# NeuralRevenant/RASSEngine

Hardware: AMD Instinct MI355X
Metric: queries/sec, exact cosine top-10 over N x 1024-d fp32 corpus in HBM (higher is better)
Workload: dtype f32; 1 GPU; 1000000 x 1024-d flat cosine top-10, 1 x MI355X, precomputed embeddings (BASELINE configs[1]); rows_per_gpu=1000000, rows_global=1000000, dim=1024, k=10, query_batch=32, corpus_dtype=f32, layout=tile16, mode=flat

## Files before the change

### include/rass_engine.h

```cpp
#ifndef RASS_ENGINE_H
#define RASS_ENGINE_H

#include <stddef.h>
#include <stdint.h>

#ifdef __cplusplus
extern "C" {
#endif

#define RASS_ABI_VERSION 1

typedef enum rass_status {
    RASS_OK = 0,
    RASS_ERR_INVALID = -1,
    RASS_ERR_HIP = -2,
    RASS_ERR_OOM = -3,
    RASS_ERR_NOT_FOUND = -4,
    RASS_ERR_UNSUPPORTED = -5,
    RASS_ERR_IO = -6
} rass_status;

typedef enum rass_dtype {
    RASS_F32 = 0,
    RASS_BF16 = 1,
// ... 304 lines not shown
                         const int64_t* d_row_ids, int64_t n, int dim, float* d_out,
                         int64_t out_stride, void* stream);
int rass_compact_plan(const int32_t* d_tags, int64_t n_rows, int64_t* d_new_row,
                      int64_t* d_src_row, int64_t* d_n_live, void* d_workspace,
                      size_t workspace_bytes, void* stream);
size_t rass_compact_plan_workspace_bytes(int64_t n_rows);
int rass_compact_rows_f32(const float* d_src, float* d_dst, int64_t row_stride,
                          const int64_t* d_src_row, int64_t n_dst, int64_t n_src_rows,
                          void* stream);

int rass_scan_topk_f32(const float* d_corpus, int64_t n_rows, int dim,
                       int64_t row_stride, const int32_t* d_row_tag,
                       const float* d_queries, int nq,
                       const int32_t* d_q_filter, int k, int64_t id_base,
                       float* d_out_scores, int64_t* d_out_ids,
                       void* d_workspace, size_t workspace_bytes,
                       void* stream);

int rass_topk_merge(const float* d_scores, const int64_t* d_ids, int n_lists,
                    int nq, int k, float* d_out_scores, int64_t* d_out_ids,
                    void* stream);

int rass_topk_merge_strided(const float* d_scores, const int64_t* d_ids,
                            int64_t score_list_stride, int64_t id_list_stride,
                            int n_lists, int nq, int k, float* d_out_scores,
                            int64_t* d_out_ids, void* stream);

int rass_topk_merge_strided_batch(const float* d_scores, const int64_t* d_ids,
                                  int64_t score_list_stride, int64_t id_list_stride,
                                  int n_lists, int nq_total, int group_size,
                                  int64_t score_group_stride, int64_t id_group_stride, int k,
                                  float* d_out_scores, int64_t* d_out_ids, void* stream);

int rass_peer_buffer_create(int device, size_t bytes, void** d_ptr, unsigned char* handle64);
int rass_peer_buffer_open(int device, const unsigned char* handle64, void** d_ptr);
int rass_peer_buffer_close(void* d_ptr, int opened_from_handle);
int rass_peer_post(const void* d_record, size_t bytes, void* d_remote_slot, void* d_remote_flag,
                   uint64_t seq, void* stream);
int rass_peer_wait(const void* d_flags, int n, int flag_stride_bytes, uint64_t seq, int* d_status,
                   int64_t max_spins, void* stream);

int rass_normalize_rows_f32(const float* d_in, int64_t in_stride, float* d_out,
                            int64_t out_stride, int64_t n, int dim,
                            void* stream);

typedef struct rass_ivf rass_ivf_t;

int rass_kmeans_assign(rass_index_t* idx, int64_t first_block, int64_t block_step,
                       int64_t n_blocks, const float* d_centroids_tile16, int nlist,
                       int32_t* d_assign, float* d_best);
int rass_kmeans_accumulate(rass_index_t* idx, int64_t first_block, int64_t block_step,
                           int64_t n_blocks, const int32_t* d_assign, float* d_sums,
                           float* d_counts, int nlist);

int rass_ivf_build(rass_index_t* src, const float* centroids, int nlist,
                   const int32_t* assign, rass_ivf_t** out);
int rass_ivf_build_ex(rass_index_t* src, const float* centroids, int nlist,
                      const int32_t* assign, rass_dtype slab_dtype, rass_ivf_t** out);
void rass_ivf_destroy(rass_ivf_t* ivf);
int rass_ivf_save(rass_ivf_t* ivf, const char* path);
int rass_ivf_load(rass_engine_t* eng, const char* path, rass_ivf_t** out);
int64_t rass_ivf_rows(const rass_ivf_t* ivf);
int rass_ivf_nlist(const rass_ivf_t* ivf);
int rass_ivf_dtype(const rass_ivf_t* ivf);
int rass_ivf_search(rass_ivf_t* ivf, const float* queries, int nq, int k,
                    int nprobe, const int32_t* q_filter, float* out_scores,
// ... 140 lines not shown
```

### rassengine_amd/_native.py

```python
from __future__ import annotations

import ctypes
import os
from typing import Optional

_HERE = os.path.dirname(os.path.abspath(__file__))
LIB_PATH = os.environ.get("RASS_HIP_LIB") or os.path.join(_HERE, "lib", "librass_hip.so")

RASS_OK = 0
RASS_MAX_K = 32
RASS_MAX_K_MULTIPASS = 4096
RASS_TAG_PATIENT_MASK = 0x00FFFFFF
RASS_TAG_DOCTYPE_SHIFT = 24
RASS_TAG_DOCTYPE_MASK = 0x7F000000
RASS_MAX_QBATCH = 32
RASS_MAX_DEVICE_BATCH = 4096
RASS_MAX_MMR_FETCH = 128
RASS_F32 = 0
RASS_BF16 = 1
RASS_QFILTER_NONE = -1
RASS_MAX_ATTRS = 8
RASS_ATTR_MISSING = -(1 << 31)
RASS_MAX_ATTR_CLAUSES = 64
RASS_ATTR_ALL, RASS_ATTR_ANY = 0, 1
# ... 170 lines not shown
                                                      ctypes.c_void_p, ctypes.c_void_p, ctypes.c_void_p]),
    "rass_index_step_floors_device": (ctypes.c_int, [ctypes.c_void_p, ctypes.c_void_p, ctypes.c_int, ctypes.c_int,
                                                     ctypes.c_void_p, ctypes.c_void_p]),
    "rass_index_save": (ctypes.c_int, [ctypes.c_void_p, ctypes.c_char_p]),
    "rass_index_load": (ctypes.c_int, [ctypes.c_void_p, ctypes.c_char_p, ctypes.c_char_p, c_void_pp]),
    "rass_index_fill_synthetic": (ctypes.c_int, [ctypes.c_void_p, ctypes.c_int64, ctypes.c_uint64,
                                                 ctypes.c_int64]),
    "rass_scan_workspace_bytes": (ctypes.c_size_t, [ctypes.c_int, ctypes.c_int]),
    "rass_scan_topk_f32": (ctypes.c_int, [ctypes.c_void_p, ctypes.c_int64, ctypes.c_int, ctypes.c_int64,
                                          ctypes.c_void_p, ctypes.c_void_p, ctypes.c_int, ctypes.c_void_p,
                                          ctypes.c_int, ctypes.c_int64, ctypes.c_void_p, ctypes.c_void_p,
                                          ctypes.c_void_p, ctypes.c_size_t, ctypes.c_void_p]),
    "rass_pack_rows_f32": (ctypes.c_int, [ctypes.c_void_p, ctypes.c_int64, ctypes.c_void_p, ctypes.c_int64,
                                          ctypes.c_int64, ctypes.c_int64, ctypes.c_int, ctypes.c_int,
                                          ctypes.c_void_p]),
    "rass_unpack_rows_f32": (ctypes.c_int, [ctypes.c_void_p, ctypes.c_int64, ctypes.c_int64, ctypes.c_int64,
                                            ctypes.c_int, ctypes.c_void_p, ctypes.c_int64, ctypes.c_void_p]),
    "rass_gather_rows_f32": (ctypes.c_int, [ctypes.c_void_p, ctypes.c_int64, ctypes.c_int64, ctypes.c_void_p, ctypes.c_int64,
                                            ctypes.c_int, ctypes.c_void_p, ctypes.c_int64, ctypes.c_void_p]),
    "rass_compact_plan": (ctypes.c_int, [ctypes.c_void_p, ctypes.c_int64, ctypes.c_void_p, ctypes.c_void_p, ctypes.c_void_p,
                                         ctypes.c_void_p, ctypes.c_size_t, ctypes.c_void_p]),
    "rass_compact_plan_workspace_bytes": (ctypes.c_size_t, [ctypes.c_int64]),
    "rass_compact_rows_f32": (ctypes.c_int, [ctypes.c_void_p, ctypes.c_void_p, ctypes.c_int64, ctypes.c_void_p, ctypes.c_int64,
                                             ctypes.c_int64, ctypes.c_void_p]),
    "rass_topk_merge": (ctypes.c_int, [ctypes.c_void_p, ctypes.c_void_p, ctypes.c_int, ctypes.c_int, ctypes.c_int,
                                       ctypes.c_void_p, ctypes.c_void_p, ctypes.c_void_p]),
    "rass_topk_merge_strided": (ctypes.c_int, [ctypes.c_void_p, ctypes.c_void_p, ctypes.c_int64, ctypes.c_int64,
                                               ctypes.c_int, ctypes.c_int, ctypes.c_int, ctypes.c_void_p,
                                               ctypes.c_void_p, ctypes.c_void_p]),
    "rass_topk_merge_strided_batch": (ctypes.c_int, [ctypes.c_void_p, ctypes.c_void_p, ctypes.c_int64, ctypes.c_int64,
                                                     ctypes.c_int, ctypes.c_int, ctypes.c_int, ctypes.c_int64,
                                                     ctypes.c_int64, ctypes.c_int, ctypes.c_void_p, ctypes.c_void_p,
                                                     ctypes.c_void_p]),
    "rass_normalize_rows_f32": (ctypes.c_int, [ctypes.c_void_p, ctypes.c_int64, ctypes.c_void_p, ctypes.c_int64,
                                               ctypes.c_int64, ctypes.c_int, ctypes.c_void_p]),
    "rass_peer_buffer_create": (ctypes.c_int, [ctypes.c_int, ctypes.c_size_t, c_void_pp, ctypes.c_char_p]),
    "rass_peer_buffer_open": (ctypes.c_int, [ctypes.c_int, ctypes.c_char_p, c_void_pp]),
    "rass_peer_buffer_close": (ctypes.c_int, [ctypes.c_void_p, ctypes.c_int]),
    "rass_peer_post": (ctypes.c_int, [ctypes.c_void_p, ctypes.c_size_t, ctypes.c_void_p, ctypes.c_void_p,
                                      ctypes.c_uint64, ctypes.c_void_p]),
    "rass_peer_wait": (ctypes.c_int, [ctypes.c_void_p, ctypes.c_int, ctypes.c_int, ctypes.c_uint64, ctypes.c_void_p,
                                      ctypes.c_int64, ctypes.c_void_p]),
    "rass_kmeans_assign": (ctypes.c_int, [ctypes.c_void_p, ctypes.c_int64, ctypes.c_int64, ctypes.c_int64,
                                          ctypes.c_void_p, ctypes.c_int, ctypes.c_void_p, ctypes.c_void_p]),
    "rass_kmeans_accumulate": (ctypes.c_int, [ctypes.c_void_p, ctypes.c_int64, ctypes.c_int64, ctypes.c_int64,
                                              ctypes.c_void_p, ctypes.c_void_p, ctypes.c_void_p, ctypes.c_int]),
    "rass_ivf_save": (ctypes.c_int, [ctypes.c_void_p, ctypes.c_char_p]),
    "rass_ivf_load": (ctypes.c_int, [ctypes.c_void_p, ctypes.c_char_p, c_void_pp]),
    "rass_ivf_build": (ctypes.c_int, [ctypes.c_void_p, ctypes.c_void_p, ctypes.c_int, ctypes.c_void_p, c_void_pp]),
    "rass_ivf_destroy": (None, [ctypes.c_void_p]),
    "rass_ivf_build_ex": (ctypes.c_int, [ctypes.c_void_p, ctypes.c_void_p, ctypes.c_int, ctypes.c_void_p, ctypes.c_int,
                                         c_void_pp]),
    "rass_ivf_dtype": (ctypes.c_int, [ctypes.c_void_p]),
    "rass_ivf_rows": (ctypes.c_int64, [ctypes.c_void_p]),
    "rass_ivf_nlist": (ctypes.c_int, [ctypes.c_void_p]),
    "rass_ivf_search": (ctypes.c_int, [ctypes.c_void_p, ctypes.c_void_p, ctypes.c_int, ctypes.c_int, ctypes.c_int,
                                       ctypes.c_void_p, ctypes.c_void_p, ctypes.c_void_p, c_i64_p]),
    "rass_ivf_search_device": (ctypes.c_int, [ctypes.c_void_p, ctypes.c_void_p, ctypes.c_int, ctypes.c_int,
                                              ctypes.c_int, ctypes.c_void_p, ctypes.c_void_p, ctypes.c_void_p]),
    "rass_ivf_search_device_batch": (ctypes.c_int, [ctypes.c_void_p, ctypes.c_void_p, ctypes.c_int, ctypes.c_int,
                                                    ctypes.c_int, ctypes.c_void_p, ctypes.c_void_p, ctypes.c_void_p,
                                                    ctypes.c_void_p]),
    "rass_ivf_build_prefix": (ctypes.c_int, [ctypes.c_void_p, ctypes.c_void_p, ctypes.c_int, ctypes.c_void_p, ctypes.c_int,
                                             ctypes.c_int64, c_void_pp]),
    "rass_ivf_covered_rows": (ctypes.c_int64, [ctypes.c_void_p]),
    "rass_ivf_delete": (ctypes.c_int, [ctypes.c_void_p, ctypes.c_int64]),
# ... 127 lines not shown
```

### rassengine_amd/csrc/api.hip

```cpp

#include "api_internal.h"

namespace rass {
namespace host {

thread_local std::string g_err;

int fail(int code, const std::string& msg) {
    g_err = msg;
    (void)hipGetLastError();
    return code;
}


int hip_fail(hipError_t e, const char* expr, const char* file, int line) {
    char b[512];
    snprintf(b, sizeof(b), "%s failed: %s (%s:%d)", expr, hipGetErrorString(e), file, line);
    return fail(e == hipErrorOutOfMemory ? RASS_ERR_OOM : RASS_ERR_HIP, b);
}

int check_nq(int nq) {
    return nq < 1 || nq > RASS_MAX_QBATCH ? fail(RASS_ERR_INVALID, "nq must be in [1, RASS_MAX_QBATCH]") : RASS_OK;
}
int check_k(int k) { return k < 1 || k > RASS_MAX_K ? fail(RASS_ERR_INVALID, "k must be in [1, RASS_MAX_K]") : RASS_OK; }
// ... 899 lines not shown
    if ((int64_t)n_lists * k > rass::kMergeMaxCandidates)
        return fail(RASS_ERR_UNSUPPORTED, "n_lists * k exceeds 8192 candidates");
    HIP_TRY(rass::launch_merge_topk(d_scores, d_ids, n_lists, nq, k, d_out_scores, d_out_ids,
                                    reinterpret_cast<hipStream_t>(stream), nullptr, score_list_stride,
                                    id_list_stride));
    return RASS_OK;
}

int rass_topk_merge_strided_batch(const float* d_scores, const int64_t* d_ids, int64_t score_list_stride,
                                  int64_t id_list_stride, int n_lists, int nq_total, int group_size,
                                  int64_t score_group_stride, int64_t id_group_stride, int k, float* d_out_scores,
                                  int64_t* d_out_ids, void* stream) {
    if (!d_scores || !d_ids || !d_out_scores || !d_out_ids) return fail(RASS_ERR_INVALID, "NULL argument");
    if (n_lists < 1 || nq_total < 1 || k < 1 || k > RASS_MAX_K || group_size < 1 || group_size > RASS_MAX_QBATCH)
        return fail(RASS_ERR_INVALID, "bad n_lists / nq_total / group_size / k");
    if (score_group_stride < (int64_t)group_size * k || id_group_stride < (int64_t)group_size * k ||
        score_list_stride < (int64_t)group_size * k || id_list_stride < (int64_t)group_size * k)
        return fail(RASS_ERR_INVALID, "list and group strides must be >= group_size * k elements");
    if ((int64_t)n_lists * k > rass::kMergeMaxCandidates)
        return fail(RASS_ERR_UNSUPPORTED, "n_lists * k exceeds 8192 candidates");
    rass::MergeGroups mg;
    mg.size = group_size;
    mg.nq_total = nq_total;
    mg.lists_are_dense = false;
    mg.score_stride = score_group_stride;
    mg.id_stride = id_group_stride;
    mg.out_score_stride = mg.out_id_stride = (int64_t)group_size * k;
    HIP_TRY(rass::launch_merge_topk(d_scores, d_ids, n_lists, nq_total, k, d_out_scores, d_out_ids,
                                    reinterpret_cast<hipStream_t>(stream), nullptr, score_list_stride, id_list_stride,
                                    &mg));
    return RASS_OK;
}

int rass_normalize_rows_f32(const float* d_in, int64_t in_stride, float* d_out, int64_t out_stride, int64_t n,
                            int dim, void* stream) {
    if (n < 0 || dim < 1 || in_stride < dim || out_stride < dim) return fail(RASS_ERR_INVALID, "bad shape");
    if (n > 0 && (!d_in || !d_out)) return fail(RASS_ERR_INVALID, "NULL argument");
    HIP_TRY(rass::launch_normalize_rows_f32(d_in, in_stride, d_out, out_stride, n, dim,
                                            reinterpret_cast<hipStream_t>(stream)));
    return RASS_OK;
}

struct rass_timer {
    hipEvent_t start = nullptr, stop = nullptr;
};

int rass_timer_create(rass_timer_t** out) {
    if (!out) return fail(RASS_ERR_INVALID, "out is NULL");
    rass_timer* t = new (std::nothrow) rass_timer();
    if (!t) return fail(RASS_ERR_OOM, "host allocation failed");
    hipError_t e = hipEventCreate(&t->start);
    if (e == hipSuccess) e = hipEventCreate(&t->stop);
    if (e != hipSuccess) {
        rass_timer_destroy(t);
        return fail(RASS_ERR_HIP, std::string("hipEventCreate: ") + hipGetErrorString(e));
    }
    *out = t;
    return RASS_OK;
}

void rass_timer_destroy(rass_timer_t* t) {
    if (!t) return;
    if (t->start) (void)hipEventDestroy(t->start);
    if (t->stop) (void)hipEventDestroy(t->stop);
    delete t;
}
// ... 182 lines not shown
```

### rassengine_amd/csrc/api_internal.h

```cpp
#pragma once

#include <hip/hip_runtime.h>
#include <stdint.h>
#include <stdio.h>
#include <stdlib.h>
#include <string.h>
#include <unistd.h>

#include <algorithm>
#include <atomic>
#include <condition_variable>
#include <map>
#include <mutex>
#include <new>
#include <string>
#include <type_traits>
#include <vector>

#include "../../include/rass_engine.h"
#include "kernels.h"

namespace rass {
namespace host {

// ... 300 lines not shown
    int64_t* d_scanned = nullptr;
    float* d_probe_scores = nullptr;
    int64_t* d_probe_ids = nullptr;
    uint32_t* d_tau = nullptr;
    uint32_t* d_list_mask = nullptr;
    bool any_tags = false;
    int64_t src_rows = 0;
    int64_t src_epoch = -1;
    std::vector<int32_t> pos_of;
    float* d_pair_scores = nullptr;
    int64_t* d_pair_ids = nullptr;
    unsigned char* d_batch = nullptr;
    size_t batch_bytes = 0;
    unsigned char* d_allow_ws = nullptr;
    size_t allow_ws_bytes = 0;
};

namespace rass {
namespace host {

int set_device(const rass_engine* eng);
int index_reserve(rass_index* idx, int64_t need_rows);
void index_free_slabs(rass_index* idx);
int index_attr_ensure(rass_index* idx, int col);
int index_refresh_copies(rass_index* idx, int64_t first, int64_t n, hipStream_t st);

int scan_xcd_skew(int nq, int grid, int n_cus);
int64_t scan_sample_floor_min_share();
bool i8_sample_floor(int64_t rows, int grid);
enum { kBatchSampleGroups = 0, kBatchSampleF32 = 1, kBatchSampleRep = 2 };
int scan_batch_sample_mode();
bool scan_batch_pair();
bool scan_batch_step();
bool ivf_batch_one_launch();

int scan_grid(int64_t tiles, int lists_kept_per_wg, int n_cus);

template <class F>
int timed_launch(rass_engine* eng, hipStream_t st, F&& launch, int extra_groups = 0) {
    const bool timed = eng && eng->ev_on && (size_t)(2 * eng->ev_used + 1) < eng->ev_pool.size();
    if (timed) HIP_TRY(hipEventRecord(eng->ev_pool[2 * eng->ev_used], st));
    const int rc = launch();
    if (rc != RASS_OK) return rc;
    if (timed) {
        HIP_TRY(hipEventRecord(eng->ev_pool[2 * eng->ev_used + 1], st));
        eng->ev_used += 1;
        eng->ev_extra += extra_groups;
    }
    return RASS_OK;
}

inline void as_sample(rass::ScanArgs& s) { s.xcd_skew = 0, s.sample_pass = true; }
inline void as_sample(rass::ScanBf16Args& s) { s.k = 1; }
inline void as_sample(rass::ScanI8Args& s) { s.k = 1; }
template <class Args>
int sample_prelaunch(Args& a, int grid, float* best, hipError_t (*launch)(const Args&, int, hipStream_t), hipStream_t st,
                     int launch_grid = 0) {
    Args s = a;
    s.n_rows = 64 * grid;
    as_sample(s);
    s.part_scores = best;
    s.part_ids = nullptr;
    HIP_TRY(launch(s, launch_grid ? launch_grid : grid, st));
    a.sample_best = best;
    a.sample_groups = grid;
    return RASS_OK;
// ... 161 lines not shown
```

### rassengine_amd/csrc/api_scan.hip

```cpp

#include "api_internal.h"

namespace rass {
namespace host {


int scan_xcd_skew(int nq, int grid, int n_cus) {
    struct Skew {
        int b16 = 4, b32 = 0;
        Skew() {
            if (const char* e = getenv("RASS_SCAN_XCD_SKEW")) {
                int a = 0, b = 0;
                const int n = sscanf(e, "%d,%d", &a, &b);
                if (n == 1) b = a;
                if (n >= 1 && a >= 0 && b >= 0 && a <= 4096 && b <= 4096) b16 = a, b32 = b;
            }
        }
    };
    if (grid != n_cus || grid % 8 != 0) return 0;
    static const Skew skew;
    return nq <= 16 ? skew.b16 : skew.b32;
}

int64_t scan_sample_floor_min_share() {
    const char* e = getenv("RASS_SCAN_SAMPLE_FLOOR");
    if (e && e[0] == '0') return 0;
    if (e && e[0] == 'f') return 2;
    return 32;
}

bool i8_sample_floor(int64_t rows, int grid) {
    const char* e = getenv("RASS_I8_SAMPLE_FLOOR");
    const bool force = e && e[0] == 'f';
    if (e && !force && atoi(e) == 0) return false;
    return grid <= rass::kMaxSampleGroups && rows >= (int64_t)(force ? 2 : 8) * 64 * grid;
}

int scan_batch_sample_mode() {
    const char* e = getenv("RASS_SCAN_BATCH_SAMPLE");
    if (e && e[0] == 'g') return kBatchSampleGroups;
    if (e && e[0] == 'f') return kBatchSampleF32;
    return kBatchSampleRep;
}

bool scan_batch_pair() {
    static const bool on = [] {
        const char* e = getenv("RASS_SCAN_BATCH_PAIR");
        return !(e && e[0] == '0');
    }();
    return on;
}

bool scan_batch_step() {
    const char* e = getenv("RASS_SCAN_BATCH_STEP");
    return !(e && e[0] == '0');
}

bool ivf_batch_one_launch() {
    const char* e = getenv("RASS_IVF_BATCH_FINE");
    return !(e && e[0] == 'g');
}


int scan_grid(int64_t tiles, int lists_kept_per_wg, int n_cus) {
    int grid = (int)std::min<int64_t>(std::max<int64_t>(tiles, 1), std::min(n_cus, kMaxGrid));
    if ((int64_t)grid * lists_kept_per_wg > rass::kMergeMaxCandidates) grid = rass::kMergeMaxCandidates / lists_kept_per_wg;
    return grid;
}

ScratchView scratch_layout(unsigned char* base, int nq, int k) {
    Carver c{base};
    ScratchView L;
    L.q_padded = c.take<float>((size_t)RASS_MAX_QBATCH * kMaxStride * sizeof(float));
    L.part_scores = c.take<float>((size_t)kMaxGrid * nq * k * sizeof(float));
    L.part_ids = c.take<int64_t>((size_t)kMaxGrid * nq * k * sizeof(int64_t));
    L.q_bf16 = c.take<unsigned short>((size_t)RASS_MAX_QBATCH * kMaxStride * 2);
    L.cand_scores = c.take<float>((size_t)RASS_MAX_QBATCH * RASS_MAX_K * sizeof(float));
    L.cand_ids = c.take<int64_t>((size_t)RASS_MAX_QBATCH * RASS_MAX_K * sizeof(int64_t));
    L.sample_best = c.take<float>((size_t)rass::kMaxSampleGroups * 32 * sizeof(float));
    L.total = c.off;
    return L;
}

BatchView batch_layout(unsigned char* base, int groups, int grid, int k, int64_t stride, bool candidates) {
    Carver c{base};
    BatchView L;
    L.part_per_group = (size_t)grid * 32 * k;
    L.q_padded = c.take<float>((size_t)groups * 32 * stride * sizeof(float));
// ... 427 lines not shown
```

### rassengine_amd/csrc/api_search.hip

```cpp

#include "api_internal.h"

namespace rass {
namespace host {

HostSlot* slot_acquire(rass_engine* eng) {
    std::unique_lock<std::mutex> lk(eng->slot_mu);
    for (;;) {
        for (HostSlot& sl : eng->slots)
            if (!sl.busy) {
                sl.busy = true;
                return &sl;
            }
        eng->slot_cv.wait(lk);
    }
}

void slot_release(rass_engine* eng, HostSlot* sl) {
    {
        std::lock_guard<std::mutex> lk(eng->slot_mu);
        sl->busy = false;
    }
    eng->slot_cv.notify_one();
}
// ... 147 lines not shown
        }
    const bool pairs = scan_batch_pair() && rass::scan_pair_supported_stride(stride);
    const int n_pairs = pairs ? nq / (2 * RASS_MAX_QBATCH) : 0;
    const bool step = scan_batch_step() && n_pairs >= 2 && grid <= (rows + 31) / 32;
    if (step && sample) HIP_TRY(rass::launch_step_floors(L.sample_best, sample_wgs, n_pairs * 64, k, L.step_floor, st));
    for (int g = 0; g < groups; ++g) {
        rass::ScanArgs a = group_args(g);
        if (sample && a.nq > 16) {
            a.sample_best = L.group_sample(g);
            a.sample_groups = sample_wgs;
        }
        const bool pair = pairs && a.nq == RASS_MAX_QBATCH && (g + 2) * RASS_MAX_QBATCH <= nq;
        const int run = pair && step ? std::min(rass::kStepMaxPairs, n_pairs - g / 2) : 1;
        if (pair) {
            a.nq = 2 * RASS_MAX_QBATCH;
            a.q_group_stride = 32 * stride;
            a.part_group_stride = (int64_t)L.part_per_group;
            a.xcd_skew = scan_xcd_skew(a.nq, grid, eng->n_cus);
        }
        if (run >= 2) {
            a.sample_best = nullptr, a.sample_groups = 0;
            a.step_floors = sample ? L.step_floor + g * 32 : nullptr;
            a.nq_total = 64 * run;
            rc = timed_launch(eng, st, [&] { return HIP_RC(rass::launch_scan_topk_f32_step(a, grid, st)); }, 2 * run - 1);
            g += 2 * run - 1;
        } else if (pair) {
            rc = timed_launch(eng, st, [&] { return HIP_RC(rass::launch_scan_topk_f32_pair(a, grid, st)); }, 1);
            ++g;
        } else
            rc = timed_launch(eng, st, [&] { return HIP_RC(rass::launch_scan_topk_f32(a, grid, st)); });
        if (rc != RASS_OK) return rc;
    }
    const rass::MergeGroups mg = dense_groups(nq, (int64_t)L.part_per_group, gs, gi);
    HIP_TRY(rass::launch_merge_topk(L.part_scores, L.part_ids, grid, nq, k, r.out_scores, r.out_ids, st, iv.id_map, 0, 0, &mg));
    return RASS_OK;
}

int sample_floor_hook(rass_index* idx, const float* d_queries, int nq, int k, const int32_t* d_q_filter, int32_t* d_rows,
                      float* d_scores, float* d_floors = nullptr) {
    rass_engine* eng = idx->eng;
    hipStream_t st = eng->stream;
    const IndexView iv = index_view(idx, d_q_filter != nullptr, 0);
    const int64_t stride = idx->stride;
    if (idx->dtype != RASS_F32 || idx->prefilter || nq <= RASS_MAX_QBATCH || iv.rows <= 0 || iv.rows > kMaxScanRows ||
        stride > kNarrowStride || !rass::scan_supported_stride(stride))
        return fail(RASS_ERR_UNSUPPORTED, "not a fused fp32 batch");
    const BatchSamplePlan plan = batch_sample_plan(eng, iv.rows, stride, nq, k);
    if (!plan.rep) return fail(RASS_ERR_UNSUPPORTED, "this batch does not take the representatives' sample stage");
    const int groups = nq / RASS_MAX_QBATCH;
    int rc = grow_block(&eng->d_batch, &eng->batch_bytes, batch_layout(nullptr, groups, plan.grid, k, stride).total, st);
    if (rc != RASS_OK) return rc;
    const BatchView L = batch_layout(eng->d_batch, groups, plan.grid, k, stride);
    HIP_TRY(rass::launch_normalize_rows_f32(d_queries, idx->dim, L.q_padded, stride, nq, idx->dim, st, nq));
    HIP_TRY(rass::launch_sample_rep(iv.corpus, iv.row_tag, stride, plan.grid, L.q_padded, d_q_filter, nq, L.rep_qfrag, L.rep_part,
                                    L.rep_row, L.sample_best, st));
    if (d_floors) {
        HIP_TRY(rass::launch_step_floors(L.sample_best, 32, nq, k, L.step_floor, st));
        HIP_TRY(hipMemcpyAsync(d_floors, L.step_floor, (size_t)nq * sizeof(float), hipMemcpyDeviceToDevice, st));
        return RASS_OK;
    }
    HIP_TRY(hipMemcpyAsync(d_rows, L.rep_row, (size_t)nq * 32 * sizeof(int32_t), hipMemcpyDeviceToDevice, st));
    HIP_TRY(hipMemcpy2DAsync(d_scores, 32 * sizeof(float), L.sample_best, rass::kMaxSampleGroups * sizeof(float), 32 * sizeof(float),
                             (size_t)nq, hipMemcpyDeviceToDevice, st));
    return RASS_OK;
}

int prefilter_launch_batch(rass_index* idx, const FlatRequest& r, int64_t gs, int64_t gi) {
// ... 414 lines not shown
```

### rassengine_amd/csrc/kernels.h

```cpp
#pragma once

#include <hip/hip_runtime.h>
#include <stddef.h>
#include <stdint.h>

namespace rass {

constexpr int kMaxSampleGroups = 256;

struct ScanArgs {
    const float* corpus;
    const int32_t* row_tag;
    const float* q_padded;
    const int32_t* q_filter;
    const int32_t* q_filter_mask = nullptr;
    const float* q_after_score = nullptr;
    const int64_t* q_after_id = nullptr;
    float* part_scores;
    int64_t* part_ids;
    int64_t row_stride;
    int64_t id_base;
    int n_rows;
    int nq;
    int k;
// ... 87 lines not shown
};
hipError_t launch_scan_fscore_f32(const FscoreArgs& a, int grid, hipStream_t stream);

struct ScoreFnRec {
    int32_t kind, col, filter, modifier;
    double weight, p0, p1, c, missing;
};
struct ScoreFnArgs {
    const int32_t* col[8] = {};
    const ScoreFnRec* recs = nullptr;
    const int32_t* q_off = nullptr;
    const uint32_t* filters = nullptr;
    int64_t words = 0;
    int64_t n_rows = 0;
    float* out = nullptr;
    int64_t stride = 0;
    int nq = 0, score_mode = 0;
    double max_boost = 0;
};
hipError_t launch_score_fn(const ScoreFnArgs& a, hipStream_t stream);

constexpr int kMergeMaxCandidates = 8192;
struct MergeGroups {
    int size = 0;
    int nq_total = 0;
    bool lists_are_dense = false;
    int64_t score_stride = 0, id_stride = 0, out_score_stride = 0, out_id_stride = 0;
};
hipError_t launch_merge_topk(const float* scores, const int64_t* ids, int n_lists, int nq, int k,
                             float* out_scores, int64_t* out_ids, hipStream_t stream,
                             const int64_t* id_map = nullptr, int64_t score_list_stride = 0,
                             int64_t id_list_stride = 0, const MergeGroups* groups = nullptr,
                             const int32_t* live_nq = nullptr);

hipError_t launch_range_finish(const unsigned* count, const uint2* hits, int nq, int cap, int64_t id_base, const int64_t* id_map,
                               float* out_scores, int64_t* out_ids, int64_t* total, hipStream_t stream);

constexpr int kGroupMaxK = 4096;
constexpr int kGroupMaxGroups = 1 << 20;
hipError_t launch_group_select(const unsigned long long* table, int nq, int n_groups, int k, int64_t id_base, const int64_t* id_map,
                               float* out_scores, int64_t* out_ids, int32_t* out_groups, int64_t* total, const unsigned* status,
                               int32_t* out_status, hipStream_t stream);
hipError_t launch_group_count_select(const unsigned* counts, const unsigned long long* best, int nq, int n_groups, int size, int64_t id_base,
                                     const int64_t* id_map, int32_t* out_groups, int64_t* out_counts, float* out_scores, int64_t* out_ids,
                                     int64_t* n_buckets, int64_t* total_hits, const unsigned* status, int32_t* out_status,
                                     hipStream_t stream);

hipError_t launch_allow_from_rows(const int64_t* rows, int64_t n, int64_t n_rows, uint32_t* allow, hipStream_t stream);
constexpr int kAllowLdsValues = 2048;
hipError_t launch_allow_from_tag_values(const int32_t* tags, int64_t n_rows, const int32_t* values, int n_values, int32_t mask,
                                        uint32_t* allow, hipStream_t stream);
size_t allow_plan_workspace_bytes(int64_t n_rows);
hipError_t launch_allow_plan(const uint32_t* allow, int64_t q_stride, int nq, int64_t n_rows, int32_t* work_tile, int32_t* work_rows,
                             uint32_t* work_mask, int32_t* n_work, void* workspace, hipStream_t stream);
hipError_t launch_allow_store(const float* scores, const int64_t* rows, int nq, int kk, int k, int kdone, int64_t id_base,
                              const int64_t* id_map, float* out_scores, int64_t* out_ids, float* after_s, int64_t* after_i,
                              hipStream_t stream);
hipError_t launch_allow_count(const uint32_t* allow, int64_t q_stride, int n_bitmaps, int64_t n_rows, int64_t* counts, hipStream_t stream);

size_t ivf_allow_workspace_bytes(int64_t max_items);
hipError_t launch_ivf_allow_words(const int32_t* work_tile, const int32_t* work_rows, uint32_t* work_mask, const int32_t* n_work,
                                  int64_t max_items, const int64_t* slab_ids, const uint32_t* allow, int64_t q_stride, int64_t words,
                                  int nq, uint32_t* slab_allow, int64_t slab_q_stride, int32_t* out_tile, int32_t* out_rows,
                                  uint32_t* out_mask, int32_t* out_n, int64_t* scanned_rows, void* workspace, hipStream_t stream);
hipError_t launch_work_rows_add(const int32_t* work_rows, const int32_t* n_work, int64_t max_items, const int64_t* add_from, int64_t* accum,
                                hipStream_t stream);
// ... 246 lines not shown
```

### rassengine_amd/csrc/merge_topk.hip

```cpp

#include <hip/hip_runtime.h>
#include <stdint.h>

#include "kernels.h"
#include "scan_core.h"

namespace rass {

constexpr int kMergeWaves = 16;
constexpr int kMergeThreads = kMergeWaves * 64;
constexpr int64_t kWorstId = 0x7fffffffffffffffLL;

struct Cand {
    float s;
    int64_t id;
};

__device__ __forceinline__ bool cand_better(const Cand& a, const Cand& b) {
    return (a.s > b.s) || (a.s == b.s && a.id < b.id);
}

template <int STRIDE>
__device__ __forceinline__ Cand xor_cand(const Cand& c, int lane) {
    Cand o;
    o.s = __int_as_float(xor_lane<STRIDE>(__float_as_int(c.s), lane));
    const int lo = xor_lane<STRIDE>((int)(c.id & 0xffffffffLL), lane);
    const int hi = xor_lane<STRIDE>((int)(c.id >> 32), lane);
    o.id = ((int64_t)hi << 32) | (uint32_t)lo;
    return o;
}

__device__ __forceinline__ Cand reverse_cand(const Cand& c, int lane) {
    Cand o = xor_cand<32>(c, lane);
    o = xor_cand<16>(o, lane);
    o.s = __int_as_float(__builtin_amdgcn_mov_dpp(__float_as_int(o.s), 0x140, 0xf, 0xf, true));
    const int lo = __builtin_amdgcn_mov_dpp((int)(o.id & 0xffffffffLL), 0x140, 0xf, 0xf, true);
    const int hi = __builtin_amdgcn_mov_dpp((int)(o.id >> 32), 0x140, 0xf, 0xf, true);
    o.id = ((int64_t)hi << 32) | (uint32_t)lo;
    return o;
}

template <int STRIDE>
__device__ __forceinline__ void cmpx(Cand& c, int lane, bool keep_better) {
    const Cand o = xor_cand<STRIDE>(c, lane);
    const bool mine_better = cand_better(c, o);
    if (mine_better != keep_better) c = o;
}

template <int SIZE, int STRIDE>
__device__ __forceinline__ void sort_steps(Cand& c, int lane) {
    if constexpr (STRIDE > 0) {
        const bool best_first = (lane & SIZE) == 0;
        const bool lower = (lane & STRIDE) == 0;
        cmpx<STRIDE>(c, lane, best_first == lower);
        sort_steps<SIZE, STRIDE / 2>(c, lane);
    }
}

__device__ __forceinline__ void wave_sort64(Cand& c, int lane) {
    sort_steps<2, 1>(c, lane);
    sort_steps<4, 2>(c, lane);
    sort_steps<8, 4>(c, lane);
    sort_steps<16, 8>(c, lane);
    sort_steps<32, 16>(c, lane);
    sort_steps<64, 32>(c, lane);
}

template <int STRIDE>
__device__ __forceinline__ void merge_steps(Cand& c, int lane) {
    if constexpr (STRIDE > 0) {
        cmpx<STRIDE>(c, lane, (lane & STRIDE) == 0);
        merge_steps<STRIDE / 2>(c, lane);
    }
}
__device__ __forceinline__ void wave_bitonic_merge64(Cand& c, int lane) { merge_steps<32>(c, lane); }

__device__ __forceinline__ void fold_group(Cand& run, const Cand& grp_sorted, int lane) {
    const Cand rev = reverse_cand(grp_sorted, lane);
    Cand c = (lane < 32) ? run : rev;
    wave_bitonic_merge64(c, lane);
    run = c;
}

__global__ __launch_bounds__(kMergeThreads) void merge_topk_kernel(const float* __restrict__ scores,
                                                                   const int64_t* __restrict__ ids, int n_lists,
                                                                   int , int k, float* __restrict__ out_scores,
                                                                   int64_t* __restrict__ out_ids,
                                                                   const int64_t* __restrict__ id_map,
                                                                   int64_t score_list_stride, int64_t id_list_stride,
                                                                   MergeGroups grp, const int32_t* __restrict__ live_nq) {
    if (live_nq != nullptr && __builtin_amdgcn_readfirstlane(*live_nq) == 0) return;
    __shared__ float sh_s[kMergeWaves * 32];
    __shared__ int64_t sh_i[kMergeWaves * 32];
    int q = blockIdx.x;
    if (grp.size > 0) {
        const int g = q / grp.size;
        q -= g * grp.size;
        scores += (int64_t)g * grp.score_stride;
        ids += (int64_t)g * grp.id_stride;
        out_scores += (int64_t)g * grp.out_score_stride;
        out_ids += (int64_t)g * grp.out_id_stride;
        if (grp.lists_are_dense) {
            const int nq_g = min(grp.size, grp.nq_total - g * grp.size);
            score_list_stride = id_list_stride = (int64_t)nq_g * k;
        }
    }
    const int lane = threadIdx.x & 63;
    const int wave = threadIdx.x >> 6;
    const int n = n_lists * k;

    Cand run;
    run.s = -INFINITY;
    run.id = kWorstId;
    for (int base = wave * 64; base < n; base += kMergeWaves * 64) {
        const int e = base + lane;
// ... 129 lines not shown
```

Before: 61330 queries/s.

## Add single-wave threshold-select top-k merge kernel and use it by default

```diff
diff --git a/include/rass_engine.h b/include/rass_engine.h
--- a/include/rass_engine.h
+++ b/include/rass_engine.h
@@ -360,6 +360,11 @@
                                   int64_t score_group_stride, int64_t id_group_stride, int k,
                                   float* d_out_scores, int64_t* d_out_ids, void* stream);
 
+int rass_topk_merge_select_device(const float* d_scores, const int64_t* d_ids, int n_lists, int nq_total, int k,
+                                  int group_size, int64_t list_group_stride, int64_t out_score_group_stride,
+                                  int64_t out_id_group_stride, float* d_out_scores, int64_t* d_out_ids,
+                                  int32_t* d_streamed, void* stream);
+
 int rass_peer_buffer_create(int device, size_t bytes, void** d_ptr, unsigned char* handle64);
 int rass_peer_buffer_open(int device, const unsigned char* handle64, void** d_ptr);
 int rass_peer_buffer_close(void* d_ptr, int opened_from_handle);
diff --git a/rassengine_amd/_native.py b/rassengine_amd/_native.py
--- a/rassengine_amd/_native.py
+++ b/rassengine_amd/_native.py
@@ -226,6 +226,9 @@
                                                      ctypes.c_int, ctypes.c_int, ctypes.c_int, ctypes.c_int64,
                                                      ctypes.c_int64, ctypes.c_int, ctypes.c_void_p, ctypes.c_void_p,
                                                      ctypes.c_void_p]),
+    "rass_topk_merge_select_device": (ctypes.c_int, [ctypes.c_void_p, ctypes.c_void_p, ctypes.c_int, ctypes.c_int, ctypes.c_int,
+                                                     ctypes.c_int, ctypes.c_int64, ctypes.c_int64, ctypes.c_int64,
+                                                     ctypes.c_void_p, ctypes.c_void_p, ctypes.c_void_p, ctypes.c_void_p]),
     "rass_normalize_rows_f32": (ctypes.c_int, [ctypes.c_void_p, ctypes.c_int64, ctypes.c_void_p, ctypes.c_int64,
                                                ctypes.c_int64, ctypes.c_int, ctypes.c_void_p]),
     "rass_peer_buffer_create": (ctypes.c_int, [ctypes.c_int, ctypes.c_size_t, c_void_pp, ctypes.c_char_p]),
diff --git a/rassengine_amd/csrc/api.hip b/rassengine_amd/csrc/api.hip
--- a/rassengine_amd/csrc/api.hip
+++ b/rassengine_amd/csrc/api.hip
@@ -955,6 +955,29 @@
     return RASS_OK;
 }
 
+int rass_topk_merge_select_device(const float* d_scores, const int64_t* d_ids, int n_lists, int nq_total, int k, int group_size,
+                                  int64_t list_group_stride, int64_t out_score_group_stride, int64_t out_id_group_stride,
+                                  float* d_out_scores, int64_t* d_out_ids, int32_t* d_streamed, void* stream) {
+    if (!d_scores || !d_ids || !d_out_scores || !d_out_ids) return fail(RASS_ERR_INVALID, "NULL argument");
+    if (n_lists < 1 || nq_total < 1 || k < 1 || k > RASS_MAX_K || group_size < 1 || group_size > RASS_MAX_QBATCH)
+        return fail(RASS_ERR_INVALID, "bad n_lists / nq_total / group_size / k");
+    if (list_group_stride < (int64_t)n_lists * group_size * k || out_score_group_stride < (int64_t)group_size * k ||
+        out_id_group_stride < (int64_t)group_size * k)
+        return fail(RASS_ERR_INVALID, "group strides must hold a full group");
+    if ((int64_t)n_lists * k > rass::kMergeMaxCandidates)
+        return fail(RASS_ERR_UNSUPPORTED, "n_lists * k exceeds 8192 candidates");
+    rass::MergeGroups mg;
+    mg.size = group_size;
+    mg.nq_total = nq_total;
+    mg.lists_are_dense = true;
+    mg.score_stride = mg.id_stride = list_group_stride;
+    mg.out_score_stride = out_score_group_stride;
+    mg.out_id_stride = out_id_group_stride;
+    HIP_TRY(rass::launch_merge_select(d_scores, d_ids, n_lists, nq_total, k, d_out_scores, d_out_ids,
+                                      reinterpret_cast<hipStream_t>(stream), nullptr, &mg, d_streamed));
+    return RASS_OK;
+}
+
 int rass_normalize_rows_f32(const float* d_in, int64_t in_stride, float* d_out, int64_t out_stride, int64_t n,
                             int dim, void* stream) {
     if (n < 0 || dim < 1 || in_stride < dim || out_stride < dim) return fail(RASS_ERR_INVALID, "bad shape");
diff --git a/rassengine_amd/csrc/api_internal.h b/rassengine_amd/csrc/api_internal.h
--- a/rassengine_amd/csrc/api_internal.h
+++ b/rassengine_amd/csrc/api_internal.h
@@ -356,6 +356,7 @@
 int scan_batch_sample_mode();
 bool scan_batch_pair();
 bool scan_batch_step();
+bool scan_batch_merge_select();
 bool ivf_batch_one_launch();
 
 int scan_grid(int64_t tiles, int lists_kept_per_wg, int n_cus);
diff --git a/rassengine_amd/csrc/api_scan.hip b/rassengine_amd/csrc/api_scan.hip
--- a/rassengine_amd/csrc/api_scan.hip
+++ b/rassengine_amd/csrc/api_scan.hip
@@ -54,6 +54,11 @@
 bool scan_batch_step() {
     const char* e = getenv("RASS_SCAN_BATCH_STEP");
     return !(e && e[0] == '0');
+}
+
+bool scan_batch_merge_select() {
+    const char* e = getenv("RASS_SCAN_BATCH_MERGE");
+    return !(e && e[0] == 's');
 }
 
 bool ivf_batch_one_launch() {
diff --git a/rassengine_amd/csrc/api_search.hip b/rassengine_amd/csrc/api_search.hip
--- a/rassengine_amd/csrc/api_search.hip
+++ b/rassengine_amd/csrc/api_search.hip
@@ -203,7 +203,10 @@
         if (rc != RASS_OK) return rc;
     }
     const rass::MergeGroups mg = dense_groups(nq, (int64_t)L.part_per_group, gs, gi);
-    HIP_TRY(rass::launch_merge_topk(L.part_scores, L.part_ids, grid, nq, k, r.out_scores, r.out_ids, st, iv.id_map, 0, 0, &mg));
+    if (scan_batch_merge_select())
+        HIP_TRY(rass::launch_merge_select(L.part_scores, L.part_ids, grid, nq, k, r.out_scores, r.out_ids, st, iv.id_map, &mg));
+    else
+        HIP_TRY(rass::launch_merge_topk(L.part_scores, L.part_ids, grid, nq, k, r.out_scores, r.out_ids, st, iv.id_map, 0, 0, &mg));
     return RASS_OK;
 }
 
diff --git a/rassengine_amd/csrc/kernels.h b/rassengine_amd/csrc/kernels.h
--- a/rassengine_amd/csrc/kernels.h
+++ b/rassengine_amd/csrc/kernels.h
@@ -143,6 +143,9 @@
                              const int64_t* id_map = nullptr, int64_t score_list_stride = 0,
                              int64_t id_list_stride = 0, const MergeGroups* groups = nullptr,
                              const int32_t* live_nq = nullptr);
+hipError_t launch_merge_select(const float* scores, const int64_t* ids, int n_lists, int nq, int k, float* out_scores,
+                               int64_t* out_ids, hipStream_t stream, const int64_t* id_map = nullptr,
+                               const MergeGroups* groups = nullptr, int32_t* streamed = nullptr);
 
 hipError_t launch_range_finish(const unsigned* count, const uint2* hits, int nq, int cap, int64_t id_base, const int64_t* id_map,
                                float* out_scores, int64_t* out_ids, int64_t* total, hipStream_t stream);
diff --git a/rassengine_amd/csrc/merge_core.h b/rassengine_amd/csrc/merge_core.h
--- /dev/null
+++ b/rassengine_amd/csrc/merge_core.h
@@ -0,0 +1,82 @@
+#pragma once
+#include <hip/hip_runtime.h>
+#include <stdint.h>
+
+#include "scan_core.h"
+
+namespace rass {
+
+constexpr int64_t kWorstId = 0x7fffffffffffffffLL;
+
+struct Cand {
+    float s;
+    int64_t id;
+};
+
+__device__ __forceinline__ bool cand_better(const Cand& a, const Cand& b) {
+    return (a.s > b.s) || (a.s == b.s && a.id < b.id);
+}
+
+template <int STRIDE>
+__device__ __forceinline__ Cand xor_cand(const Cand& c, int lane) {
+    Cand o;
+    o.s = __int_as_float(xor_lane<STRIDE>(__float_as_int(c.s), lane));
+    const int lo = xor_lane<STRIDE>((int)(c.id & 0xffffffffLL), lane);
+    const int hi = xor_lane<STRIDE>((int)(c.id >> 32), lane);
+    o.id = ((int64_t)hi << 32) | (uint32_t)lo;
+    return o;
+}
+
+__device__ __forceinline__ Cand reverse_cand(const Cand& c, int lane) {
+    Cand o = xor_cand<32>(c, lane);
+    o = xor_cand<16>(o, lane);
+    o.s = __int_as_float(__builtin_amdgcn_mov_dpp(__float_as_int(o.s), 0x140, 0xf, 0xf, true));
+    const int lo = __builtin_amdgcn_mov_dpp((int)(o.id & 0xffffffffLL), 0x140, 0xf, 0xf, true);
+    const int hi = __builtin_amdgcn_mov_dpp((int)(o.id >> 32), 0x140, 0xf, 0xf, true);
+    o.id = ((int64_t)hi << 32) | (uint32_t)lo;
+    return o;
+}
+
+template <int STRIDE>
+__device__ __forceinline__ void cmpx(Cand& c, int lane, bool keep_better) {
+    const Cand o = xor_cand<STRIDE>(c, lane);
+    const bool mine_better = cand_better(c, o);
+    if (mine_better != keep_better) c = o;
+}
+
+template <int SIZE, int STRIDE>
+__device__ __forceinline__ void sort_steps(Cand& c, int lane) {
+    if constexpr (STRIDE > 0) {
+        const bool best_first = (lane & SIZE) == 0;
+        const bool lower = (lane & STRIDE) == 0;
+        cmpx<STRIDE>(c, lane, best_first == lower);
+        sort_steps<SIZE, STRIDE / 2>(c, lane);
+    }
+}
+
+__device__ __forceinline__ void wave_sort64(Cand& c, int lane) {
+    sort_steps<2, 1>(c, lane);
+    sort_steps<4, 2>(c, lane);
+    sort_steps<8, 4>(c, lane);
+    sort_steps<16, 8>(c, lane);
+    sort_steps<32, 16>(c, lane);
+    sort_steps<64, 32>(c, lane);
+}
+
+template <int STRIDE>
+__device__ __forceinline__ void merge_steps(Cand& c, int lane) {
+    if constexpr (STRIDE > 0) {
+        cmpx<STRIDE>(c, lane, (lane & STRIDE) == 0);
+        merge_steps<STRIDE / 2>(c, lane);
+    }
+}
+__device__ __forceinline__ void wave_bitonic_merge64(Cand& c, int lane) { merge_steps<32>(c, lane); }
+
+__device__ __forceinline__ void fold_group(Cand& run, const Cand& grp_sorted, int lane) {
+    const Cand rev = reverse_cand(grp_sorted, lane);
+    Cand c = (lane < 32) ? run : rev;
+    wave_bitonic_merge64(c, lane);
+    run = c;
+}
+
+}
diff --git a/rassengine_amd/csrc/merge_select.hip b/rassengine_amd/csrc/merge_select.hip
--- /dev/null
+++ b/rassengine_amd/csrc/merge_select.hip
@@ -0,0 +1,134 @@
+
+#include <hip/hip_runtime.h>
+#include <stdint.h>
+
+#include "kernels.h"
+#include "merge_core.h"
+
+namespace rass {
+
+constexpr int kSelectBuf = 256;
+constexpr int kXcds = 8;
+constexpr int kSelectAhead = 8;
+
+__global__ __launch_bounds__(64) void merge_select_kernel(const float* __restrict__ scores, const int64_t* __restrict__ ids,
+                                                          int n_lists, int k, float* __restrict__ out_scores,
+                                                          int64_t* __restrict__ out_ids, const int64_t* __restrict__ id_map,
+                                                          int64_t score_list_stride, int64_t id_list_stride, MergeGroups grp,
+                                                          int32_t* __restrict__ streamed) {
+    __shared__ float sh_s[kSelectBuf];
+    __shared__ int64_t sh_i[kSelectBuf];
+    const int nq_all = gridDim.x, xcd = blockIdx.x % kXcds, per = nq_all / kXcds, rem = nq_all % kXcds;
+    int q = xcd * per + min(xcd, rem) + blockIdx.x / kXcds;
+    if (grp.size > 0) {
+        const int g = q / grp.size;
+        q -= g * grp.size;
+        scores += (int64_t)g * grp.score_stride;
+        ids += (int64_t)g * grp.id_stride;
+        out_scores += (int64_t)g * grp.out_score_stride;
+        out_ids += (int64_t)g * grp.out_id_stride;
+        if (grp.lists_are_dense) {
+            const int nq_g = min(grp.size, grp.nq_total - g * grp.size);
+            score_list_stride = id_list_stride = (int64_t)nq_g * k;
+        }
+    }
+    const int lane = threadIdx.x;
+    const int n = n_lists * k;
+    const unsigned inv_k = ((1u << 18) + (unsigned)k - 1u) / (unsigned)k;
+    const int64_t qo = (int64_t)q * k;
+
+    auto load = [&](int e) {
+        const int ee = min(e, n - 1);
+        const int list = (int)(((unsigned)ee * inv_k) >> 18), kk = ee - list * k;
+        const int64_t gi = ids[(int64_t)list * id_list_stride + qo + kk];
+        const float gs = scores[(int64_t)list * score_list_stride + qo + kk];
+        const bool valid = e < n && gi >= 0 && gs > -INFINITY;
+        Cand c;
+        c.s = valid ? gs : -INFINITY;
+        c.id = valid ? gi : kWorstId;
+        return c;
+    };
+    auto slot = [&](int base) { return base + ((lane + (base >> 6)) & 63); };
+
+    Cand best;
+    best.s = -INFINITY;
+    best.id = kWorstId;
+    for (int base = 0; base < n; base += 64 * kSelectAhead) {
+        Cand c[kSelectAhead];
+#pragma unroll
+        for (int u = 0; u < kSelectAhead; ++u) c[u] = load(slot(base + 64 * u));
+#pragma unroll
+        for (int u = 0; u < kSelectAhead; ++u)
+            if (cand_better(c[u], best)) best = c[u];
+    }
+    wave_sort64(best, lane);
+    Cand T;
+    T.s = __shfl(best.s, k - 1);
+    T.id = ((int64_t)__shfl((int)(best.id >> 32), k - 1) << 32) | (uint32_t)__shfl((int)(best.id & 0xffffffffLL), k - 1);
+
+    int cnt = 0;
+    for (int base = 0; base < n; base += 64 * kSelectAhead) {
+        Cand c[kSelectAhead];
+#pragma unroll
+        for (int u = 0; u < kSelectAhead; ++u) c[u] = load(slot(base + 64 * u));
+#pragma unroll
+        for (int u = 0; u < kSelectAhead; ++u) {
+            const bool keep = c[u].s > -INFINITY && !cand_better(T, c[u]);
+            const unsigned long long mask = __ballot(keep);
+            const int at = cnt + __popcll(mask & ((1ull << lane) - 1ull));
+            if (keep && at < kSelectBuf) {
+                sh_s[at] = c[u].s;
+                sh_i[at] = c[u].id;
+            }
+            cnt += __popcll(mask);
+        }
+    }
+    __syncthreads();
+
+    const bool stream = cnt > kSelectBuf;
+    if (stream && streamed != nullptr && lane == 0) atomicAdd(streamed, 1);
+    const int total = stream ? n : cnt;
+    Cand run;
+    run.s = -INFINITY;
+    run.id = kWorstId;
+    for (int base = 0; base < total; base += 64) {
+        Cand c;
+        if (stream)
+            c = load(base + lane);
+        else {
+            c.s = -INFINITY;
+            c.id = kWorstId;
+            if (base + lane < cnt) {
+                c.s = sh_s[base + lane];
+                c.id = sh_i[base + lane];
+            }
+        }
+        wave_sort64(c, lane);
+        if (base == 0)
+            run = c;
+        else
+            fold_group(run, c, lane);
+    }
+    if (lane < k) {
+        const bool filled = run.id != kWorstId;
+        out_scores[qo + lane] = filled ? run.s : -INFINITY;
+        out_ids[qo + lane] = filled ? (id_map ? id_map[run.id] : run.id) : (int64_t)-1;
+    }
+}
+
+hipError_t launch_merge_select(const float* scores, const int64_t* ids, int n_lists, int nq, int k, float* out_scores,
+                               int64_t* out_ids, hipStream_t stream, const int64_t* id_map, const MergeGroups* groups,
+                               int32_t* streamed) {
+    const int64_t n = (int64_t)n_lists * k;
+    if (n_lists < 1 || nq < 1 || k < 1 || k > 32 || n > kMergeMaxCandidates) return hipErrorInvalidValue;
+    MergeGroups grp;
+    if (groups) {
+        grp = *groups;
+        if (grp.size < 1 || grp.nq_total != nq) return hipErrorInvalidValue;
+    }
+    hipLaunchKernelGGL(merge_select_kernel, dim3(nq), dim3(64), 0, stream, scores, ids, n_lists, k, out_scores, out_ids, id_map,
+                       (int64_t)nq * k, (int64_t)nq * k, grp, streamed);
+    return hipGetLastError();
+}
+
+}
diff --git a/rassengine_amd/csrc/merge_topk.hip b/rassengine_amd/csrc/merge_topk.hip
--- a/rassengine_amd/csrc/merge_topk.hip
+++ b/rassengine_amd/csrc/merge_topk.hip
@@ -3,84 +3,12 @@
 #include <stdint.h>
 
 #include "kernels.h"
-#include "scan_core.h"
+#include "merge_core.h"
 
 namespace rass {
 
 constexpr int kMergeWaves = 16;
 constexpr int kMergeThreads = kMergeWaves * 64;
-constexpr int64_t kWorstId = 0x7fffffffffffffffLL;
-
-struct Cand {
-    float s;
-    int64_t id;
-};
-
-__device__ __forceinline__ bool cand_better(const Cand& a, const Cand& b) {
-    return (a.s > b.s) || (a.s == b.s && a.id < b.id);
-}
-
-template <int STRIDE>
-__device__ __forceinline__ Cand xor_cand(const Cand& c, int lane) {
-    Cand o;
-    o.s = __int_as_float(xor_lane<STRIDE>(__float_as_int(c.s), lane));
-    const int lo = xor_lane<STRIDE>((int)(c.id & 0xffffffffLL), lane);
-    const int hi = xor_lane<STRIDE>((int)(c.id >> 32), lane);
-    o.id = ((int64_t)hi << 32) | (uint32_t)lo;
-    return o;
-}
-
-__device__ __forceinline__ Cand reverse_cand(const Cand& c, int lane) {
-    Cand o = xor_cand<32>(c, lane);
-    o = xor_cand<16>(o, lane);
-    o.s = __int_as_float(__builtin_amdgcn_mov_dpp(__float_as_int(o.s), 0x140, 0xf, 0xf, true));
-    const int lo = __builtin_amdgcn_mov_dpp((int)(o.id & 0xffffffffLL), 0x140, 0xf, 0xf, true);
-    const int hi = __builtin_amdgcn_mov_dpp((int)(o.id >> 32), 0x140, 0xf, 0xf, true);
-    o.id = ((int64_t)hi << 32) | (uint32_t)lo;
-    return o;
-}
-
-template <int STRIDE>
-__device__ __forceinline__ void cmpx(Cand& c, int lane, bool keep_better) {
-    const Cand o = xor_cand<STRIDE>(c, lane);
-    const bool mine_better = cand_better(c, o);
-    if (mine_better != keep_better) c = o;
-}
-
-template <int SIZE, int STRIDE>
-__device__ __forceinline__ void sort_steps(Cand& c, int lane) {
-    if constexpr (STRIDE > 0) {
-        const bool best_first = (lane & SIZE) == 0;
-        const bool lower = (lane & STRIDE) == 0;
-        cmpx<STRIDE>(c, lane, best_first == lower);
-        sort_steps<SIZE, STRIDE / 2>(c, lane);
-    }
-}
-
-__device__ __forceinline__ void wave_sort64(Cand& c, int lane) {
-    sort_steps<2, 1>(c, lane);
-    sort_steps<4, 2>(c, lane);
-    sort_steps<8, 4>(c, lane);
-    sort_steps<16, 8>(c, lane);
-    sort_steps<32, 16>(c, lane);
-    sort_steps<64, 32>(c, lane);
-}
-
-template <int STRIDE>
-__device__ __forceinline__ void merge_steps(Cand& c, int lane) {
-    if constexpr (STRIDE > 0) {
-        cmpx<STRIDE>(c, lane, (lane & STRIDE) == 0);
-        merge_steps<STRIDE / 2>(c, lane);
-    }
-}
-__device__ __forceinline__ void wave_bitonic_merge64(Cand& c, int lane) { merge_steps<32>(c, lane); }
-
-__device__ __forceinline__ void fold_group(Cand& run, const Cand& grp_sorted, int lane) {
-    const Cand rev = reverse_cand(grp_sorted, lane);
-    Cand c = (lane < 32) ? run : rev;
-    wave_bitonic_merge64(c, lane);
-    run = c;
-}
 
 __global__ __launch_bounds__(kMergeThreads) void merge_topk_kernel(const float* __restrict__ scores,
                                                                    const int64_t* __restrict__ ids, int n_lists,
```

Measured after the change: 61470 queries/s, median of 6. About the same (+0.2%).
